# Lab-LVM/imagenet-models

Measured on AMD Instinct MI355X. Metric: images/sec (whole node) GA-ConvNeXt-T 3x224x224 bf16 training step, higher is better.
Workload: dtype bf16; 1 GPU; ga_convnext_tiny_768 train step (fwd + GA loss lam=-0.8 + bwd + all-reduce + adamw lr=0), batch 256/GPU, drop_path 0.2, synthetic 3x224x224; global_batch=256, parallelism=dp1, dist_backend=none, grad_exchange=torch, allreduce_buckets=0

## Files before the change

imagenet-models_amd/_lib.py:

```python
import ctypes as C
import os

_HERE = os.path.dirname(os.path.abspath(__file__))
LIB_PATH = os.environ.get('GAEXT_LIB') or os.path.join(_HERE, 'csrc', 'libgaext.so')

GA_F32, GA_BF16 = 0, 1
ACT_NONE, ACT_GELU, ACT_RELU = 0, 1, 2
A_PLAIN, A_PATCH2, A_STEM4_NCHW, A_CONV3, A_CONV3S2, A_NEIGH2 = 0, 1, 2, 3, 4, 5
C_PLAIN, C_UNPATCH2 = 0, 1

vp, i32, i64, f32 = C.c_void_p, C.c_int, C.c_int64, C.c_float


class GemmDesc(C.Structure):
    _fields_ = [
        ('M', i32), ('N', i32), ('K', i32), ('batch', i32), ('dtype', i32),
        ('A', vp), ('lda', i64), ('strideA', i64), ('a_batch_mod', i32), ('a_kind', i32),
        ('a_H', i32), ('a_W', i32), ('a_C', i32), ('a_act', i32),
        ('B', vp), ('ldb', i64), ('strideB', i64),
        ('C', vp), ('ldc', i64), ('strideC', i64), ('c_kind', i32),
        ('c_H', i32), ('c_W', i32), ('c_C', i32), ('c_f32', i32), ('C2', vp), ('c2_mode', i32),
        ('alpha', f32), ('bias', vp), ('strideBias', i64), ('act', i32),
        ('H', vp), ('ldh', i64), ('strideH', i64), ('h_is_deriv', i32),
        ('rowscale', vp), ('rows_per_scale', i32),
# ... 82 lines not shown
    'ga_unset_knob': ([C.c_char_p], i32),
    'ga_config_string': ([C.c_char_p, C.c_size_t], i32),
    'ga_gemm': ([C.POINTER(GemmDesc), vp], i32),
    'ga_wgrad': ([C.POINTER(WgradDesc), vp], i32),
    'ga_weight_prep': ([C.POINTER(WprepDesc), vp], i32),
    'ga_bias_fold': ([vp, vp, vp, vp, vp, vp, i32, i32, vp], i32),
    'ga_weight_unfold': ([C.POINTER(WunfoldDesc), vp], i32),
    'ga_dwconv7_fwd': ([vp, vp, vp, vp, i32, i32, i32, i32, i32, vp], i32),
    'ga_dwconv7_bwd_data': ([vp, vp, vp, vp, i32, i32, i32, i32, i32, vp], i32),
    'ga_dwconv7_bwd_data2': ([vp, vp, vp, vp, vp, vp, i32, i32, i32, i32, i32, vp], i32),
    'ga_dwconv7_bwd_weight': ([vp, vp, vp, vp, i32, i32, i32, i32, i32, vp, C.c_size_t, vp], i32),
    'ga_dwconv7_bwd_weight_workspace': ([i32, i32, i32, i32, i32], C.c_size_t),
    'ga_dwconv3_fwd': ([vp, vp, vp, i32, i32, i32, i32, i32, vp, vp, i32, vp], i32),
    'ga_dwconv3_bwd_data': ([vp, vp, vp, i32, i32, i32, i32, i32, i32, vp], i32),
    'ga_dwconv3_bwd_weight': ([vp, vp, vp, i32, i32, i32, i32, i32, i32, vp, C.c_size_t, vp], i32),
    'ga_dwconv3_bwd_weight_workspace': ([i32, i32, i32, i32, i32, i32], C.c_size_t),
    'ga_maxpool3s2_fwd': ([vp, vp, vp, i32, i32, i32, i32, i32, vp], i32),
    'ga_maxpool3s2_bwd': ([vp, vp, vp, i32, i32, i32, i32, i32, i32, vp], i32),
    'ga_bn_gelu_fwd': ([vp, vp, vp, vp, i64, i32, i32, vp], i32),
    'ga_bn_gelu_bwd_workspace': ([i64, i32], C.c_size_t),
    'ga_bn_gelu_bwd_reduce': ([vp, vp, vp, vp, vp, vp, vp, vp, i64, i32, i32, vp, C.c_size_t, vp], i32),
    'ga_bn_gelu_bwd_apply': ([vp, vp, vp, vp, vp, vp, vp, vp, vp, i64, vp, i64, i32, i32, vp], i32),
    'ga_se_bn_fwd': ([vp, i32, vp, vp, vp, vp, vp, vp, vp, vp, vp, vp, vp, vp, vp, vp, i32, i32, i32, i32, vp], i32),
    'ga_se_bn_bwd': ([vp, vp, vp, vp, vp, vp, vp, vp, i32, vp, vp, vp, vp, vp, vp, vp, vp, vp, vp, vp, vp, vp, vp, vp, vp, vp, vp, vp,
                      vp, vp, i32, i32, i32, vp], i32),
    'ga_se_residual_fwd': ([vp, vp, vp, vp, vp, vp, vp, vp, vp, i32, i32, i32, i32, vp], i32),
    'ga_se_residual_bwd_a': ([vp, vp, vp, vp, vp, vp, vp, vp, i32, i32, i32, i32, vp], i32),
    'ga_se_residual_bwd_b': ([vp, vp, vp, vp, vp, vp, vp, vp, vp, vp, vp, i32, i32, i32, i32, vp], i32),
    'ga_subsample2_fwd': ([vp, vp, i32, i32, i32, i32, i32, vp], i32),
    'ga_subsample2_bwd': ([vp, vp, i32, i32, i32, i32, i32, i32, vp], i32),
    'ga_wgrad_workspace': ([C.POINTER(WgradDesc)], C.c_size_t),
    'ga_gemm_form': ([C.POINTER(GemmDesc), C.c_char_p, C.c_size_t], i32),
    'ga_wgrad_form': ([C.POINTER(WgradDesc), C.c_char_p, C.c_size_t], i32),
    'ga_layernorm_fwd': ([vp, vp, vp, vp, vp, vp, i64, i32, f32, i32, vp], i32),
    'ga_layernorm_bwd': ([vp, vp, vp, vp, vp, vp, vp, vp, vp, i64, i32, i32, i32, vp], i32),
    'ga_layernorm_bwd_dp': ([vp, vp, vp, vp, vp, vp, vp, vp, vp, i64, i32, i32, vp, vp, i64, i32, vp], i32),
    'ga_bn_finalize': ([vp, vp, i64, vp, vp, f32, f32, vp, vp, vp, vp, vp, vp, i32, i32, vp], i32),
    'ga_affine_act': ([vp, vp, vp, vp, vp, i64, vp, i64, i32, i32, i32, i64, vp], i32),
    'ga_bn_bwd_reduce': ([vp, vp, vp, vp, vp, vp, i64, vp, vp, i64, i32, i32, i64, vp], i32),
    'ga_bn_bwd_apply': ([vp, vp, vp, vp, vp, vp, vp, vp, vp, i64, i64, vp, i64, i32, i32, i64, i64, vp], i32),
    'ga_pool_concat_fwd': ([vp, vp, i32, i32, i32, i32, i32, i32, i32, i32, i32, i32, vp], i32),
    'ga_pool_concat_bwd': ([vp, vp, vp, i32, i32, i32, i32, i32, i32, i32, i32, i32, i32, vp], i32),
    'ga_spatial_sum': ([vp, vp, vp, i32, i32, i32, f32, i32, vp], i32),
    'ga_se_mlp_fwd': ([vp, vp, vp, vp, vp, vp, vp, i32, i32, i32, vp], i32),
    'ga_se_mlp_bwd': ([vp, vp, vp, vp, vp, vp, vp, f32, vp, vp, vp, vp, i32, i32, i32, vp], i32),
    'ga_chan_scale': ([vp, vp, vp, vp, i32, i32, i32, i32, vp], i32),
    'ga_gram_pack_fwd': ([vp, vp, vp, i32, i32, i32, i32, i32, vp], i32),
    'ga_gram_pack_bwd': ([vp, vp, vp, vp, i32, i32, i32, i32, i32, vp], i32),
    'ga_gram_f64_fwd_workspace': ([i32, i32], C.c_size_t),
    'ga_gram_f64_bwd_workspace': ([i32, i32], C.c_size_t),
    'ga_gram_f64_fwd': ([vp, vp, vp, vp, C.c_size_t, i32, i32, i32, i32, i32, i32, i32, vp], i32),
    'ga_gram_f64_bwd': ([vp, vp, vp, vp, vp, vp, C.c_size_t, i32, i32, i32, i32, i32, i32, i32, vp], i32),
    'ga_token_cat': ([vp, vp, vp, i32, i32, i32, i32, vp], i32),
    'ga_token_split': ([vp, vp, vp, i32, i32, i32, i32, i32, i32, vp], i32),
    'ga_class_attn_fwd': ([vp, vp, vp, vp, i32, i32, i32, i32, f32, i32, vp], i32),
    'ga_class_attn_bwd': ([vp, vp, vp, vp, vp, vp, i32, i32, i32, i32, f32, i32, vp], i32),
    'ga_class_attn_fwd2': ([vp, vp, vp, i64, vp, vp, i32, i32, i32, i32, f32, i32, vp], i32),
    'ga_class_attn_bwd2': ([vp, vp, vp, vp, i64, vp, vp, vp, vp, i32, i32, i32, i32, f32, i32, vp], i32),
    'ga_loss_fwd_bwd': ([vp, vp, vp, vp, i32, i32, i32, f32, i32, f32, f32, i32, vp], i32),
    'ga_heads_topk': ([vp, i32, i32, i32, i32, vp, vp, vp], i32),
    'ga_sgd_step': ([vp, vp, vp, vp, i64, i32, f32, vp], i32),
    'ga_adamw_step': ([vp, vp, vp, vp, vp, i64, f32, vp], i32),
    'ga_weight_prep_batch': ([vp, i32, vp], i32),
    'ga_weight_unfold_batch': ([vp, i32, vp], i32),
    'ga_small_batch': ([vp, i32, vp], i32),
    'ga_cswin_attn_fwd': ([C.POINTER(CswinAttnDesc), vp], i32),
# ... 157 lines not shown
```

imagenet-models_amd/csrc/gemm.hip:

```cpp
#include <stdlib.h>
#include <algorithm>
#include <type_traits>
#include "common.h"
#include "gemm_select.h"

namespace {

constexpr int kThreads = 256;
constexpr int kRowBytes = 128;

__device__ __forceinline__ int xcd_remap(int bid, int nwg) {
    const int q = nwg >> 3, r = nwg & 7, xcd = bid & 7, idx = bid >> 3;
    return (xcd < r ? xcd * (q + 1) : r * (q + 1) + (xcd - r) * q) + idx;
}

struct RowCtx {
    long base;
    int y, x;
    bool valid;
};

__device__ __forceinline__ RowCtx make_row(int kind, long m, long M, long ld, int H, int W, int C) {
    RowCtx r;
    r.valid = m < M;
// ... 1717 lines not shown
                }
            }
    if (do_bias) {
#pragma unroll
        for (int tn = 0; tn < 8; ++tn) {
            float v = bsum[tn];
            v += __shfl_xor(v, 16, 64);
            v += __shfl_xor(v, 32, 64);
            const int n = n0 + wn * 128 + tn * 16 + lane;
            if (lane < 16 && n < d.N) atomicAdd(d.dbias + z * d.strideDbias + n, v * d.alpha);
        }
    }
}

__global__ __launch_bounds__(256) void tn2_reduce_kernel(const float* __restrict__ part, int nsplit, long nk, int K,
                                                         float alpha, float* __restrict__ dW, long ldw, long strideW) {
    const long z = blockIdx.y;
    const float* p = part + z * nsplit * nk;
    for (long i = ((long)blockIdx.x * 256 + threadIdx.x) * 4; i < nk; i += (long)gridDim.x * 1024) {
        float4 a = *reinterpret_cast<const float4*>(p + i);
#pragma unroll 4
        for (int s = 1; s < nsplit; ++s) {
            const float4 b = *reinterpret_cast<const float4*>(p + (long)s * nk + i);
            a.x += b.x; a.y += b.y; a.z += b.z; a.w += b.w;
        }
        const long n = i / K, k = i - n * K;
        float* dst = dW + z * strideW + n * ldw + k;
        dst[0] += alpha * a.x; dst[1] += alpha * a.y; dst[2] += alpha * a.z; dst[3] += alpha * a.w;
    }
}

using namespace gasel;

Knobs current_knobs() {
    Knobs k;
#define GA_SEL_KNOB(NAME) k.NAME = GA_KNOB(#NAME, Knobs{}.NAME)
    GA_SEL_KNOB(NT_R3); GA_SEL_KNOB(NT_R3_NEIGH2); GA_SEL_KNOB(NT_R3_CONV3S2); GA_SEL_KNOB(NT_PP); GA_SEL_KNOB(NT_PP_MINK);
    GA_SEL_KNOB(NT_BIG); GA_SEL_KNOB(NT_DMA); GA_SEL_KNOB(NT_DMA2); GA_SEL_KNOB(NT_DMA2_MINK); GA_SEL_KNOB(NT_T256);
    GA_SEL_KNOB(TN2); GA_SEL_KNOB(TN2_PATCH2); GA_SEL_KNOB(TN2_WGS); GA_SEL_KNOB(TN2_PART_MIN);
    GA_SEL_KNOB(CONV3_DIRECT); GA_SEL_KNOB(CONV0_DIRECT); GA_SEL_KNOB(STEM4_WGRAD_DIRECT);
#undef GA_SEL_KNOB
    return k;
}

int lds_error(int bytes) {
    ga_set_error("ga_gemm: cannot reserve %d bytes of LDS", bytes);
    return GA_ERR_HIP;
}

template <typename T, int TNW, int NWM, bool PLAIN, bool PRE, int EPI, bool DMA = false>
int launch_nt_(const ga_gemm_desc* d, hipStream_t s) {
    using CF = NTCfg<TNW, NWM>;
    constexpr int smem = DMA ? CF::SMEM_DMA : CF::SMEM;
    auto kern = gemm_nt_kernel<T, TNW, NWM, PLAIN, PRE, EPI, DMA>;
    static const int per_cu = [&] {
        int n = 0;
        if (smem > 65536 && hipFuncSetAttribute(reinterpret_cast<const void*>(kern),
                                                hipFuncAttributeMaxDynamicSharedMemorySize, smem) != hipSuccess)
            return 0;
        if (hipOccupancyMaxActiveBlocksPerMultiprocessor(&n, kern, CF::NTHR, smem) != hipSuccess || n < 1) n = 1;
        return n;
    }();
    if (per_cu == 0) return lds_error(smem);
    const int tiles = cdiv(d->M, CF::BM) * cdiv(d->N, CF::BN);
    const int cap = std::max(8, (per_cu * ga_num_cus() / d->batch) / 8 * 8);
    dim3 grid(std::min(tiles, cap), 1, d->batch), block(CF::NTHR);
    hipLaunchKernelGGL(kern, grid, block, smem, s, *d);
    return ga_check_launch("ga_gemm");
}

template <int EPI>
int launch_nt_pp(const ga_gemm_desc* d, hipStream_t s) {
    auto kern = gemm_nt_pp_kernel<EPI>;
    static const bool ok = hipFuncSetAttribute(reinterpret_cast<const void*>(kern), hipFuncAttributeMaxDynamicSharedMemorySize, kPPSmem) == hipSuccess;
    if (!ok) return lds_error(kPPSmem);
    const int tiles = cdiv(d->M, 256) * cdiv(d->N, 256);
// ... 174 lines not shown
```

imagenet-models_amd/csrc/gemm_select.h:

```cpp
#pragma once
#include <stddef.h>
#include <stdint.h>
#include <stdio.h>
#include <algorithm>
#include "../../include/gaext.h"

void ga_set_error(const char* fmt, ...);
bool ga_conv3_c64_eligible(const ga_gemm_desc* d);
bool ga_conv0_c8_eligible(const ga_gemm_desc* d);
int ga_conv3_c64_wgrad_wgs(const ga_wgrad_desc* d, int num_cus);
int ga_conv3s2_c64_wgrad_wgs(const ga_wgrad_desc* d, int num_cus);
int ga_conv0_c8_wgrad_wgs(const ga_wgrad_desc* d, int num_cus);
int ga_stem4_wgrad_wgs(const ga_wgrad_desc* d, int num_cus);

namespace gasel {

enum { EPI_GENERIC = -1, EPI_PLAIN = 0, EPI_FC1 = 1, EPI_FC2 = 2, EPI_DG2 = 3 };

struct Knobs {
    int NT_R3 = -1, NT_R3_NEIGH2 = 1, NT_R3_CONV3S2 = 1, NT_PP = -1, NT_PP_MINK = 512, NT_BIG = -1, NT_DMA = 1, NT_DMA2 = 10,
        NT_DMA2_MINK = 256, NT_T256 = -1;
    int TN2 = 1, TN2_PATCH2 = 1, TN2_WGS = 0, TN2_PART_MIN = 65536;
    int CONV3_DIRECT = 1, CONV0_DIRECT = 1, STEM4_WGRAD_DIRECT = 1;
};

inline int ceil_div(long a, long b) { return (int)((a + b - 1) / b); }
inline uintptr_t addr(const void* p) { return reinterpret_cast<uintptr_t>(p); }
inline bool aligned16(const void* p) { return (addr(p) & 15) == 0; }

#define GA_SEL_REQUIRE(cond, ...) \
    do { if (!(cond)) { ga_set_error(__VA_ARGS__); return GA_ERR_BAD_ARG; } } while (0)

inline int nt_validate(const ga_gemm_desc* d) {
    GA_SEL_REQUIRE(d && d->A && d->B && d->C, "ga_gemm: null operand");
    GA_SEL_REQUIRE(d->M > 0 && d->N > 0 && d->K > 0 && d->batch >= 1, "ga_gemm: bad shape M=%d N=%d K=%d batch=%d", d->M,
                   d->N, d->K, d->batch);
    GA_SEL_REQUIRE(d->dtype == GA_F32 || d->dtype == GA_BF16, "ga_gemm: bad dtype %d", d->dtype);
    const int epc = d->dtype == GA_BF16 ? 8 : 4;
    GA_SEL_REQUIRE(aligned16(d->A) && aligned16(d->B) && aligned16(d->C), "ga_gemm: operands must be 16-byte aligned");
    GA_SEL_REQUIRE(d->ldb % epc == 0 && d->strideB % epc == 0, "ga_gemm: ldb/strideB must be multiples of %d", epc);
    GA_SEL_REQUIRE(d->K % epc == 0, "ga_gemm: K=%d must be a multiple of %d (pad the operand)", d->K, epc);
    if (d->a_kind == GA_A_PLAIN) {
        GA_SEL_REQUIRE(d->lda % epc == 0 && d->strideA % epc == 0, "ga_gemm: lda/strideA must be multiples of %d", epc);
    } else if (d->a_kind == GA_A_PATCH2) {
        GA_SEL_REQUIRE(d->a_C % epc == 0 && d->a_H % 2 == 0 && d->a_W % 2 == 0 && d->K == 4 * d->a_C &&
                           (long)d->M % ((d->a_H / 2) * (d->a_W / 2)) == 0,
                       "ga_gemm: PATCH2 needs C%%%d==0, even H,W, K==4C", epc);
    } else if (d->a_kind == GA_A_CONV3) {
        GA_SEL_REQUIRE(d->a_C % epc == 0 && d->K == 9 * d->a_C && (long)d->M % (d->a_H * d->a_W) == 0,
                       "ga_gemm: CONV3 needs C%%%d==0, K==9C", epc);
    } else if (d->a_kind == GA_A_CONV3S2) {
        GA_SEL_REQUIRE(d->a_C % epc == 0 && d->K == 9 * d->a_C && (long)d->M % (((d->a_H + 1) / 2) * ((d->a_W + 1) / 2)) == 0,
                       "ga_gemm: CONV3S2 needs C%%%d==0, K==9C", epc);
    } else if (d->a_kind == GA_A_NEIGH2) {
        GA_SEL_REQUIRE(d->a_C % epc == 0 && d->K == 4 * d->a_C && (long)d->M % (d->a_H * d->a_W) == 0,
                       "ga_gemm: NEIGH2 needs C%%%d==0, K==4C", epc);
    } else if (d->a_kind == GA_A_STEM4_NCHW) {
// ... 206 lines not shown
    const long nk = (long)d->N * d->K;
    const long nk_min = k.TN2_PART_MIN;
    return (split > 1 && nk >= nk_min) ? (size_t)d->batch * split * nk * sizeof(float) : 0;
}

inline TnSel tn_select(const ga_wgrad_desc* d, int num_cus, const Knobs& k) {
    const bool has_ws = d->workspace != nullptr;
    int wgs;
    size_t need;
    auto direct = [&](int form, size_t per_wg) -> TnSel {
        need = (size_t)wgs * per_wg * sizeof(float);
        if (has_ws && (size_t)d->ws_bytes >= need) return {form, wgs, need, true};
        return {TN_TN, d->split_m, need, false};
    };
    if (k.CONV3_DIRECT && (wgs = ga_conv3_c64_wgrad_wgs(d, num_cus))) return direct(TN_CONV3_DIRECT, 64 * 576);
    if (k.CONV3_DIRECT && (wgs = ga_conv3s2_c64_wgrad_wgs(d, num_cus))) return direct(TN_CONV3S2_DIRECT, 64 * 576);
    if (k.CONV0_DIRECT && (wgs = ga_conv0_c8_wgrad_wgs(d, num_cus))) return direct(TN_CONV0_DIRECT, 64 * 72);
    if (k.STEM4_WGRAD_DIRECT && (wgs = ga_stem4_wgrad_wgs(d, num_cus))) return direct(TN_STEM4_DIRECT, (size_t)d->N * 49);
    if (tn2_eligible(d, k)) {
        int split;
        need = tn2_plan(d, num_cus, k, &split);
        return {TN_TN2, split, need, need && has_ws && (size_t)d->ws_bytes >= need};
    }
    return {TN_TN, d->split_m, 0, false};
}

inline void tn_form_name(const ga_wgrad_desc* d, const TnSel& s, char* buf, size_t n) {
    const char* const form[] = {"conv3_wgrad_direct", "conv3s2_wgrad_direct", "conv0_wgrad_direct", "stem4_wgrad_direct", "tn2", "tn"};
    if (s.form == TN_TN) snprintf(buf, n, "tn");
    else if (s.form != TN_TN2) snprintf(buf, n, "%s:wgs%d", form[s.form], s.split);
    else snprintf(buf, n, "tn2%s:split%d:%s", d->x_kind == GA_A_PATCH2 ? "p" : "", s.split, s.partials ? "partials" : "atomics");
}

#undef GA_SEL_REQUIRE

}
```

imagenet-models_amd/ops.py:

```python
import ctypes as C
import numbers
import os

import torch

from . import _lib as L
from ._lib import (A_CONV3, A_CONV3S2, A_NEIGH2, A_PATCH2, A_PLAIN, A_STEM4_NCHW, ACT_GELU, ACT_NONE, ACT_RELU, C_PLAIN, C_UNPATCH2,
                   GA_BF16, GA_F32)


def ga_dtype(t):
    if isinstance(t, torch.dtype):
        dt = t
    else:
        dt = t.dtype
    if dt == torch.bfloat16:
        return GA_BF16
    if dt == torch.float32:
        return GA_F32
    raise TypeError(f'unsupported dtype {dt}')


def torch_dtype(ga):
    return torch.bfloat16 if ga == GA_BF16 else torch.float32
# ... 291 lines not shown
        if apend:
            ajoin()

    def __len__(self):
        return len(self.calls)

    def mark(self, name):
        self.marks[name] = len(self.calls)

    def run_range(self, start, end, stream=None):
        self.finalize()
        s = current_stream_ptr() if stream is None else stream
        if any(self.lanes[start:end]):
            return self._run_lanes(start, end)
        for fn, args, label in self.calls[start:end]:
            rc = fn(*args, s)
            if rc != 0:
                L.check(rc, f'{self.name}:{label}')

    def gemm(self, A, B, Cout, M, N, K, dtype, lda=None, ldb=None, ldc=None, batch=1, strideA=0, strideB=0, strideC=0,
             a_batch_mod=0, a_kind=A_PLAIN, a_dims=(0, 0, 0), a_act=ACT_NONE, c_kind=C_PLAIN, c_dims=(0, 0, 0),
             c_f32=False, alpha=1.0, bias=None, strideBias=0, act=ACT_NONE, H=None, ldh=0, strideH=0, rowscale=None,
             rows_per_scale=1, R=None, ldr=0, strideR=0, relu_after=False, colsum=None, colsumsq=None, strideCol=0,
             C2=None, c2_mode=0, h_is_deriv=False, label=None):
        d = _set(L.GemmDesc(), M=M, N=N, K=K, batch=batch, dtype=dtype,
                 A=A, lda=(K if lda is None else lda), strideA=strideA, a_batch_mod=a_batch_mod, a_kind=a_kind, a_act=a_act,
                 B=B, ldb=(K if ldb is None else ldb), strideB=strideB,
                 C=Cout, ldc=(N if ldc is None else ldc), strideC=strideC, c_kind=c_kind, c_f32=c_f32, C2=C2, c2_mode=c2_mode,
                 h_is_deriv=h_is_deriv, alpha=alpha, bias=bias, strideBias=strideBias, act=act, H=H, ldh=ldh, strideH=strideH,
                 rowscale=rowscale, rows_per_scale=rows_per_scale, R=R, ldr=ldr, strideR=strideR, relu_after=relu_after,
                 colsum=colsum, colsumsq=colsumsq, strideCol=strideCol)
        d.a_H, d.a_W, d.a_C = a_dims
        d.c_H, d.c_W, d.c_C = c_dims
        self.record('ga_gemm', d, label=label)

    def attn_desc(self, qkv, out, lse, B, N, H, hd, scale, dtype, ldq=None, ldo=None):
        return _set(L.AttnDesc(), B=B, N=N, H=H, hd=hd, scale=scale, dtype=dtype, qkv=qkv, ldq=(3 * H * hd if ldq is None else ldq),
                    out=out, ldo=(H * hd if ldo is None else ldo), lse=lse)

    def attn_fwd(self, d, label=None):
        self.record('ga_attn_fwd', d, label=label)

    def attn_bwd(self, d, dout, dqkv, ws, label=None):
        self.record('ga_attn_bwd', d, dout, dqkv, ws, _nbytes(ws), label=label)

    def patchify(self, x, out, P, dtype, label=None):
        B, CH, H, W = x.shape
        self.record('ga_patchify', x, out, B, CH, H, W, P, dtype, label=label)

    def patchify_strided(self, x, out, P, S, dtype, label=None):
        B, CH, H, W = x.shape
        self.record('ga_patchify_strided', x, out, B, CH, H, W, P, S, dtype, label=label)

    def pos_add_fwd(self, tok, pos, x0, B, Np, Cdim, dtype, label=None):
        self.record('ga_pos_add_fwd', tok, pos, x0, B, Np, Cdim, dtype, label=label)

    def pos_add_bwd(self, dx0, dpos, B, Np, Cdim, dtype, label=None):
        self.record('ga_pos_add_bwd', dx0, dpos, B, Np, Cdim, dtype, label=label)

    def dwpool_fwd(self, x, w, bias, y, B, H, W_, Cin, mult, dtype, label=None):
        self.record('ga_dwpool_fwd', x, w, bias, y, B, H, W_, Cin, mult, dtype, label=label)

    def dwpool_bwd_data(self, dy, w, dx, B, H, W_, Cin, mult, dtype, label=None):
        self.record('ga_dwpool_bwd_data', dy, w, dx, B, H, W_, Cin, mult, dtype, label=label)

    def dwpool_bwd_weight(self, dy, x, dw, db, B, H, W_, Cin, mult, dtype, label=None):
        self.record('ga_dwpool_bwd_weight', dy, x, dw, db, B, H, W_, Cin, mult, dtype, label=label)
# ... 52 lines not shown
    def mlp_fwd(self, X, W1, b1, W2, b2, Y, M, Cdim, dtype, ldw1=None, ldw2=None, R=None, rowscale=None, rows_per_scale=1, label=None):
        H = 4 * Cdim
        d = _set(L.MlpDesc(), X=X, ldx=Cdim, W1=W1, ldw1=(Cdim if ldw1 is None else ldw1), b1=b1, W2=W2, ldw2=(H if ldw2 is None else ldw2),
                 b2=b2, R=R, ldr=Cdim, rowscale=rowscale, rows_per_scale=rows_per_scale, Y=Y, ldy=Cdim, M=M, C=Cdim, H=H, dtype=dtype)
        self.record('ga_mlp_fwd', d, label=label)

    def mlp_bwd(self, X, DY, W1, b1, W2T, W1T, A, DH, DX, M, Cdim, dtype, ldw1=None, ldw2t=None, ldw1t=None, label=None,
                dW1=None, db1=None, partials=None, max_blocks=0):
        H = 4 * Cdim
        d = _set(L.MlpBwdDesc(), X=X, ldx=Cdim, DY=DY, lddy=Cdim, W1=W1, ldw1=(Cdim if ldw1 is None else ldw1), b1=b1,
                 W2T=W2T, ldw2t=(Cdim if ldw2t is None else ldw2t), W1T=W1T, ldw1t=(H if ldw1t is None else ldw1t),
                 A=A, lda=H, DH=DH, lddh=H, DX=DX, lddx=Cdim, M=M, C=Cdim, H=H, dtype=dtype)
        if dW1 is not None:
            assert dW1.dtype == torch.float32 and db1 is not None and db1.dtype == torch.float32 and partials is not None
            assert dW1.stride(-1) == 1 and partials.dtype == torch.float32 and partials.is_contiguous()
            _set(d, dW1=dW1, ldw=dW1.stride(0), db1=db1, partials=partials, partials_bytes=partials.numel() * 4, max_blocks=max_blocks)
        self.record('ga_mlp_bwd', d, label=label)

    def wgrad(self, Y, X, dW, M, N, K, dtype, ldy=None, ldx=None, ldw=None, batch=1, strideY=0, strideX=0, strideW=0,
              x_kind=A_PLAIN, x_dims=(0, 0, 0), x_act=ACT_NONE, dbias=None, strideDbias=0, alpha=1.0, split_m=None,
              accumulate=True, x_batch_mod=0, label=None):
        if split_m is None:
            split_m = pick_split_m(M, N, K, batch, dtype)
        d = _set(L.WgradDesc(), M=M, N=N, K=K, batch=batch, dtype=dtype, Y=Y, ldy=(N if ldy is None else ldy), strideY=strideY,
                 X=X, ldx=(K if ldx is None else ldx), strideX=strideX, x_kind=x_kind, x_batch_mod=x_batch_mod, x_act=x_act,
                 dW=dW, ldw=(K if ldw is None else ldw), strideW=strideW, dbias=dbias, strideDbias=strideDbias, alpha=alpha,
                 split_m=split_m, accumulate=accumulate)
        d.x_H, d.x_W, d.x_C = x_dims
        need = self.lib.ga_wgrad_workspace(C.byref(d))
        if need:
            def patch(ptr, nbytes, d=d):
                d.workspace, d.ws_bytes = ptr, nbytes
            self._want_workspace(int(need), patch)
        self.record('ga_wgrad', d, label=label)

    def weight_prep(self, w, G, Co, Ci, KH, KW, dtype, out=None, ldo=0, outT=None, ldt=0, rs=None, cs=None, flip=False,
                    stem=False, row_perm=None, t_cols=0, label=None):
        d = _set(L.WprepDesc(), w=w, G=G, Co=Co, Ci=Ci, KH=KH, KW=KW, rs=rs, cs=cs, row_perm=row_perm, dtype=dtype,
                 out=out, ldo=ldo, outT=outT, ldt=ldt, flip=flip, stem=stem, t_cols=t_cols)
        if self.defer:
            return self._defer('wprep', d)
        self.record('ga_weight_prep', d, label=label)

    def bias_fold(self, W, b, rs, v, be, N, Cdim, row_perm=None, label=None):
        if self.defer:
            return self._small(kind=2, y=be, x=W, R=N, C=Cdim, b=b, rs=rs, v=v, row_perm=row_perm)
        self.record('ga_bias_fold', W, b, rs, v, row_perm, be, N, Cdim, label=label)

    def weight_unfold(self, G, ldg, N, Ci, KH=1, KW=1, gb=None, W=None, b=None, rs=None, cs=None, v=None, stem=False, dW=None,
                      db=None, d_rs=None, d_cs=None, d_v=None, row_perm=None, label=None):
        d = _set(L.WunfoldDesc(), G=G, ldg=ldg, gb=gb, W=W, b=b, rs=rs, cs=cs, v=v, row_perm=row_perm, N=N, Ci=Ci, KH=KH, KW=KW,
                 stem=stem, dW=dW, db=db, d_rs=d_rs, d_cs=d_cs, d_v=d_v)
        if self.defer:
            return self._defer('unfold', d)
        self.record('ga_weight_unfold', d, label=label)

    def dwconv7_fwd(self, x, w49, bias, y, B, H, W, Cdim, dtype, label=None):
        self.record('ga_dwconv7_fwd', x, w49, bias, y, B, H, W, Cdim, dtype, label=label)

    def dwconv7_bwd_data(self, dy, w49, res, dx, B, H, W, Cdim, dtype, dx2=None, scale2=None, label=None):
        if dx2 is not None:
            return self.record('ga_dwconv7_bwd_data2', dy, w49, res, dx, dx2, scale2, B, H, W, Cdim, dtype, label=label)
        self.record('ga_dwconv7_bwd_data', dy, w49, res, dx, B, H, W, Cdim, dtype, label=label)

    def dwconv7_bwd_weight(self, dy, x, dw49, dbias, B, H, W, Cdim, dtype, label=None):
        need = int(self.lib.ga_dwconv7_bwd_weight_workspace(B, H, W, Cdim, dtype))
        self._record_ws('ga_dwconv7_bwd_weight', need, dy, x, dw49, dbias, B, H, W, Cdim, dtype, label=label)
# ... 316 lines not shown
    def cast_to_f32(self, src, dst, n, dtype, label=None):
        self.record('ga_cast_to_f32', src, dst, n, dtype, label=label)

    def zero(self, t, label=None):
        self.record('ga_memset', t, 0, _nbytes(t), label=label or 'zero')


def mlp_supported(Cdim, H, dtype):
    return bool(L.load().ga_mlp_supported(Cdim, H, dtype))


def mlp_bwd_wgrad_supported(Cdim, H, dtype):
    return bool(L.load().ga_mlp_bwd_wgrad_supported(Cdim, H, dtype))


def mlp_bwd_partials(M, Cdim, dtype, max_blocks=0):
    d = L.MlpBwdDesc()
    d.M, d.C, d.H, d.dtype, d.max_blocks = M, Cdim, 4 * Cdim, dtype, max_blocks
    return int(L.load().ga_mlp_bwd_partials(C.byref(d)))


def gemm_form(d):
    buf = C.create_string_buffer(64)
    L.check(L.load().ga_gemm_form(C.byref(d), buf, 64), 'ga_gemm_form')
    return buf.value.decode()


def wgrad_form(d):
    buf = C.create_string_buffer(64)
    L.check(L.load().ga_wgrad_form(C.byref(d), buf, 64), 'ga_wgrad_form')
    return buf.value.decode()


def cswin_attn_bwd_workspace(d):
    return int(L.load().ga_cswin_attn_bwd_workspace(C.byref(d)))


def zero_(t):
    L.check(L.load().ga_memset(_ptr(t), 0, t.numel() * t.element_size(), current_stream_ptr()), 'ga_memset')
    return t


_NUM_CU = None


def num_cus():
    global _NUM_CU
    if _NUM_CU is None:
        n = C.c_int(256)
        L.check(L.load().ga_device_info(C.byref(n), None, None), 'ga_device_info')
        _NUM_CU = n.value
    return _NUM_CU


def pick_split_m(M, N, K, batch, dtype):
    slab = 64 if dtype == GA_BF16 else 32
    tiles = ((N + 127) // 128) * ((K + 127) // 128) * batch
    want = max(1, (2 * 256) // tiles)
    return int(max(1, min(want, (M + 4 * slab - 1) // (4 * slab))))
```

include/gaext.h:

```cpp
#ifndef GAEXT_H
#define GAEXT_H
#include <stddef.h>
#include <stdint.h>

#ifdef __cplusplus
extern "C" {
#endif

typedef void* ga_stream_t;

enum { GA_F32 = 0, GA_BF16 = 1 };
enum { GA_OK = 0, GA_ERR_BAD_ARG = -1, GA_ERR_UNSUPPORTED = -2, GA_ERR_HIP = -3 };

enum { GA_ACT_NONE = 0, GA_ACT_GELU = 1, GA_ACT_RELU = 2 };

enum {
    GA_A_PLAIN = 0,
    GA_A_PATCH2 = 1,
    GA_A_STEM4_NCHW = 2,
    GA_A_CONV3 = 3,
    GA_A_CONV3S2 = 4,
    GA_A_NEIGH2 = 5
};
enum {
// ... 43 lines not shown
    float* colsum;
    float* colsumsq;
    int64_t strideCol;
} ga_gemm_desc;
int ga_gemm(const ga_gemm_desc* d, ga_stream_t stream);

typedef struct {
    int M, N, K;
    int batch;
    int dtype;
    const void* Y;
    int64_t ldy, strideY;
    const void* X;
    int64_t ldx, strideX;
    int x_batch_mod;
    int x_kind;
    int x_H, x_W, x_C;
    int x_act;
    float* dW;
    int64_t ldw, strideW;
    float* dbias;
    int64_t strideDbias;
    float alpha;
    int split_m;
    int accumulate;
    void* workspace;
    int64_t ws_bytes;
} ga_wgrad_desc;
int ga_wgrad(const ga_wgrad_desc* d, ga_stream_t stream);
size_t ga_wgrad_workspace(const ga_wgrad_desc* d);

int ga_gemm_form(const ga_gemm_desc* d, char* buf, size_t n);
int ga_wgrad_form(const ga_wgrad_desc* d, char* buf, size_t n);

typedef struct {
    const float* w;
    int G, Co, Ci, KH, KW;
    const float* rs;
    const float* cs;
    const int* row_perm;
    int dtype;
    void* out;  int64_t ldo;
    void* outT; int64_t ldt;
    int flip;
    int stem;
    int t_cols;
} ga_wprep_desc;
int ga_weight_prep(const ga_wprep_desc* d, ga_stream_t stream);
int ga_bias_fold(const float* W, const float* b, const float* rs, const float* v, const int* row_perm, float* be, int N,
                 int C, ga_stream_t stream);
typedef struct {
    const float* G; int64_t ldg;
    const float* gb;
    const float* W; const float* b;
    const float* rs; const float* cs; const float* v;
    const int* row_perm;
    int N, Ci, KH, KW;
    int stem;
    float* dW; float* db; float* d_rs; float* d_cs; float* d_v;
} ga_wunfold_desc;
int ga_weight_unfold(const ga_wunfold_desc* d, ga_stream_t stream);

int ga_dwconv7_fwd(const void* x, const float* w49, const float* bias, void* y, int B, int H, int W, int C,
                   int dtype, ga_stream_t stream);
int ga_dwconv7_bwd_data(const void* dy, const float* w49, const void* res, void* dx, int B, int H, int W, int C,
                        int dtype, ga_stream_t stream);
// ... 328 lines not shown
```

Before: 10920 images/sec.

## Add split-K few-row GEMM and wgrad kernels for small-M launches

Adds dedicated bf16 NT and TN kernels for GEMMs with few rows (M up to 512). The NT kernel splits K across four waves and reduces partial sums in LDS; the TN kernel uses 64x64 output tiles. Both are selected only when the regular tiling would fill less than half the CUs, to raise parallelism for small head-layer GEMMs. The trade-off is an extra kernel path, extra host-side form queries while recording, and reliance on atomics for the column-sum and bias reductions.

```diff
diff --git a/imagenet-models_amd/_lib.py b/imagenet-models_amd/_lib.py
--- a/imagenet-models_amd/_lib.py
+++ b/imagenet-models_amd/_lib.py
@@ -138,6 +138,10 @@
     'ga_wgrad_workspace': ([C.POINTER(WgradDesc)], C.c_size_t),
     'ga_gemm_form': ([C.POINTER(GemmDesc), C.c_char_p, C.c_size_t], i32),
     'ga_wgrad_form': ([C.POINTER(WgradDesc), C.c_char_p, C.c_size_t], i32),
+    'ga_gemm_fewrows': ([C.POINTER(GemmDesc), vp], i32),
+    'ga_wgrad_fewrows': ([C.POINTER(WgradDesc), vp], i32),
+    'ga_gemm_fewrows_form': ([C.POINTER(GemmDesc), C.c_char_p, C.c_size_t], i32),
+    'ga_wgrad_fewrows_form': ([C.POINTER(WgradDesc), C.c_char_p, C.c_size_t], i32),
     'ga_layernorm_fwd': ([vp, vp, vp, vp, vp, vp, i64, i32, f32, i32, vp], i32),
     'ga_layernorm_bwd': ([vp, vp, vp, vp, vp, vp, vp, vp, vp, i64, i32, i32, i32, vp], i32),
     'ga_layernorm_bwd_dp': ([vp, vp, vp, vp, vp, vp, vp, vp, vp, i64, i32, i32, vp, vp, i64, i32, vp], i32),
diff --git a/imagenet-models_amd/csrc/gemm.hip b/imagenet-models_amd/csrc/gemm.hip
--- a/imagenet-models_amd/csrc/gemm.hip
+++ b/imagenet-models_amd/csrc/gemm.hip
@@ -1773,16 +1773,20 @@
 
 using namespace gasel;
 
-Knobs current_knobs() {
+}
+
+gasel::Knobs gasel::current_knobs() {
     Knobs k;
 #define GA_SEL_KNOB(NAME) k.NAME = GA_KNOB(#NAME, Knobs{}.NAME)
     GA_SEL_KNOB(NT_R3); GA_SEL_KNOB(NT_R3_NEIGH2); GA_SEL_KNOB(NT_R3_CONV3S2); GA_SEL_KNOB(NT_PP); GA_SEL_KNOB(NT_PP_MINK);
     GA_SEL_KNOB(NT_BIG); GA_SEL_KNOB(NT_DMA); GA_SEL_KNOB(NT_DMA2); GA_SEL_KNOB(NT_DMA2_MINK); GA_SEL_KNOB(NT_T256);
     GA_SEL_KNOB(TN2); GA_SEL_KNOB(TN2_PATCH2); GA_SEL_KNOB(TN2_WGS); GA_SEL_KNOB(TN2_PART_MIN);
-    GA_SEL_KNOB(CONV3_DIRECT); GA_SEL_KNOB(CONV0_DIRECT); GA_SEL_KNOB(STEM4_WGRAD_DIRECT);
+    GA_SEL_KNOB(CONV3_DIRECT); GA_SEL_KNOB(CONV0_DIRECT); GA_SEL_KNOB(STEM4_WGRAD_DIRECT); GA_SEL_KNOB(FEWROWS); GA_SEL_KNOB(FEWROWS_MAXM);
 #undef GA_SEL_KNOB
     return k;
 }
+
+namespace {
 
 int lds_error(int bytes) {
     ga_set_error("ga_gemm: cannot reserve %d bytes of LDS", bytes);
diff --git a/imagenet-models_amd/csrc/gemm_fewrows.hip b/imagenet-models_amd/csrc/gemm_fewrows.hip
--- /dev/null
+++ b/imagenet-models_amd/csrc/gemm_fewrows.hip
@@ -0,0 +1,365 @@
+#include <algorithm>
+#include "common.h"
+#include "gemm_select.h"
+
+namespace {
+
+using namespace gasel;
+
+constexpr int kFrThreads = 256;
+constexpr int kFrChunk = 4;
+
+__device__ __forceinline__ uint4 fr_zero4() { return make_uint4(0u, 0u, 0u, 0u); }
+
+struct FrFrag {
+    uint4 a[2][kFrChunk], b[2][kFrChunk];
+};
+
+__global__ __launch_bounds__(kFrThreads) void gemm_nt_fewrows_kernel(const ga_gemm_desc d) {
+    __shared__ __attribute__((aligned(16))) float part[4][32 * 32];
+    const int tid = threadIdx.x, lane = tid & 63, wave = tid >> 6;
+    const int tiles_n = (d.N + 31) >> 5;
+    const int tile_m = blockIdx.x / tiles_n, tile_n = blockIdx.x - tile_m * tiles_n;
+    const int m0 = tile_m * 32, n0 = tile_n * 32;
+    const long z = blockIdx.z;
+    const long za = d.a_batch_mod > 0 ? z % d.a_batch_mod : z;
+    const bf16_t* Ab = reinterpret_cast<const bf16_t*>(d.A) + za * d.strideA;
+    const bf16_t* Bb = reinterpret_cast<const bf16_t*>(d.B) + z * d.strideB;
+
+    const int fr = lane & 15, kq = (lane >> 4) * 8;
+    const bf16_t* Ap[2];
+    const bf16_t* Bp[2];
+#pragma unroll
+    for (int i = 0; i < 2; ++i) {
+        Ap[i] = Ab + (long)min(m0 + 16 * i + fr, d.M - 1) * d.lda;
+        Bp[i] = Bb + (long)min(n0 + 16 * i + fr, d.N - 1) * d.ldb;
+    }
+    const int nsteps = (d.K + 31) >> 5, per = (nsteps + 3) >> 2;
+    const int s0 = wave * per, s1 = min(s0 + per, nsteps);
+    const int nchunks = s1 > s0 ? (s1 - s0 + kFrChunk - 1) / kFrChunk : 0;
+
+    auto load = [&](int c, FrFrag& f) {
+#pragma unroll
+        for (int i = 0; i < kFrChunk; ++i) {
+            const int s = s0 + c * kFrChunk + i, k = s * 32 + kq;
+            const bool ok = s < s1 && k < d.K;
+            const int kk = ok ? k : 0;
+#pragma unroll
+            for (int j = 0; j < 2; ++j) {
+                const uint4 va = *reinterpret_cast<const uint4*>(Ap[j] + kk);
+                const uint4 vb = *reinterpret_cast<const uint4*>(Bp[j] + kk);
+                f.a[j][i] = ok ? va : fr_zero4();
+                f.b[j][i] = ok ? vb : fr_zero4();
+            }
+        }
+    };
+    f32x4_t acc[2][2];
+#pragma unroll
+    for (int i = 0; i < 2; ++i)
+#pragma unroll
+        for (int j = 0; j < 2; ++j) acc[i][j] = f32x4_t{0.f, 0.f, 0.f, 0.f};
+    auto mma = [&](const FrFrag& f) {
+#pragma unroll
+        for (int i = 0; i < kFrChunk; ++i)
+#pragma unroll
+            for (int bn = 0; bn < 2; ++bn)
+#pragma unroll
+                for (int bm = 0; bm < 2; ++bm)
+                    acc[bn][bm] = __builtin_amdgcn_mfma_f32_16x16x32_bf16(*reinterpret_cast<const bf16x8_t*>(&f.b[bn][i]),
+                                                                          *reinterpret_cast<const bf16x8_t*>(&f.a[bm][i]),
+                                                                          acc[bn][bm], 0, 0, 0);
+    };
+    FrFrag f0, f1;
+    if (nchunks > 0) load(0, f0);
+    for (int c = 0; c < nchunks; c += 2) {
+        if (c + 1 < nchunks) load(c + 1, f1);
+        mma(f0);
+        if (c + 1 < nchunks) {
+            if (c + 2 < nchunks) load(c + 2, f0);
+            mma(f1);
+        }
+    }
+
+#pragma unroll
+    for (int bn = 0; bn < 2; ++bn)
+#pragma unroll
+        for (int bm = 0; bm < 2; ++bm) {
+            const int row = bm * 16 + (lane & 15), c4 = bn * 4 + (lane >> 4);
+            *reinterpret_cast<f32x4_t*>(&part[wave][row * 32 + ((c4 ^ (row & 7)) << 2)]) = acc[bn][bm];
+        }
+    __syncthreads();
+
+    const int row = tid >> 3, c4 = tid & 7;
+    const long m = m0 + row;
+    const int n = n0 + c4 * 4;
+    float v[4];
+    {
+        const int o = row * 32 + ((c4 ^ (row & 7)) << 2);
+        const f32x4_t p0 = *reinterpret_cast<const f32x4_t*>(&part[0][o]), p1 = *reinterpret_cast<const f32x4_t*>(&part[1][o]);
+        const f32x4_t p2 = *reinterpret_cast<const f32x4_t*>(&part[2][o]), p3 = *reinterpret_cast<const f32x4_t*>(&part[3][o]);
+#pragma unroll
+        for (int j = 0; j < 4; ++j) v[j] = (p0[j] + p1[j]) + (p2[j] + p3[j]);
+    }
+    const bool live = m < d.M && n < d.N;
+    const bool full = n + 3 < d.N;
+    float cs[4] = {0.f, 0.f, 0.f, 0.f}, cq[4] = {0.f, 0.f, 0.f, 0.f};
+    if (live) {
+        const float* bias = d.bias ? d.bias + z * d.strideBias : nullptr;
+#pragma unroll
+        for (int j = 0; j < 4; ++j) v[j] = v[j] * d.alpha + ((bias && n + j < d.N) ? bias[n + j] : 0.f);
+        const long coff = z * d.strideC + m * d.ldc + n;
+        if (d.act == GA_ACT_GELU) {
+            float w[4];
+#pragma unroll
+            for (int j = 0; j < 4; ++j) gelu_both_fast(v[j], v[j], w[j]);
+            if (d.C2) {
+                bf16_t* C2p = reinterpret_cast<bf16_t*>(d.C2) + coff;
+                if (full) {
+                    store4(C2p, w);
+                } else {
+#pragma unroll
+                    for (int j = 0; j < 4; ++j)
+                        if (n + j < d.N) C2p[j] = f2bf(w[j]);
+                }
+            }
+        }
+        if (d.H) {
+            const bf16_t* Hp = reinterpret_cast<const bf16_t*>(d.H) + z * d.strideH + m * d.ldh + n;
+            float h[4] = {0.f, 0.f, 0.f, 0.f};
+            if (full) {
+                load4(Hp, h);
+            } else {
+#pragma unroll
+                for (int j = 0; j < 4; ++j)
+                    if (n + j < d.N) h[j] = bf2f(Hp[j]);
+            }
+#pragma unroll
+            for (int j = 0; j < 4; ++j) v[j] *= h[j];
+        }
+        if (d.rowscale) {
+            const float s = d.rowscale[(unsigned)m / (unsigned)d.rows_per_scale];
+#pragma unroll
+            for (int j = 0; j < 4; ++j) v[j] *= s;
+        }
+        if (d.R) {
+            const bf16_t* Rp = reinterpret_cast<const bf16_t*>(d.R) + z * d.strideR + m * d.ldr + n;
+            float r[4] = {0.f, 0.f, 0.f, 0.f};
+            if (full) {
+                load4(Rp, r);
+            } else {
+#pragma unroll
+                for (int j = 0; j < 4; ++j)
+                    if (n + j < d.N) r[j] = bf2f(Rp[j]);
+            }
+#pragma unroll
+            for (int j = 0; j < 4; ++j) v[j] += r[j];
+        }
+#pragma unroll
+        for (int j = 0; j < 4; ++j)
+            if (n + j < d.N) {
+                cs[j] = v[j];
+                cq[j] = v[j] * v[j];
+            }
+        if (d.c_f32) {
+            float* Cp = reinterpret_cast<float*>(d.C) + coff;
+            if (full) {
+                store4(Cp, v);
+            } else {
+#pragma unroll
+                for (int j = 0; j < 4; ++j)
+                    if (n + j < d.N) Cp[j] = v[j];
+            }
+        } else {
+            bf16_t* Cp = reinterpret_cast<bf16_t*>(d.C) + coff;
+            if (full) {
+                store4(Cp, v);
+            } else {
+#pragma unroll
+                for (int j = 0; j < 4; ++j)
+                    if (n + j < d.N) Cp[j] = f2bf(v[j]);
+            }
+        }
+    }
+    if (d.colsum) {
+        const bool sq = d.colsumsq != nullptr;
+#pragma unroll
+        for (int j = 0; j < 4; ++j) {
+#pragma unroll
+            for (int o = 8; o < 64; o <<= 1) {
+                cs[j] += __shfl_xor(cs[j], o, 64);
+                cq[j] += __shfl_xor(cq[j], o, 64);
+            }
+        }
+        __syncthreads();
+        float* red = &part[0][0];
+        if (lane < 8) {
+#pragma unroll
+            for (int j = 0; j < 4; ++j) {
+                red[wave * 32 + lane * 4 + j] = cs[j];
+                red[128 + wave * 32 + lane * 4 + j] = cq[j];
+            }
+        }
+        __syncthreads();
+        if (tid < 64) {
+            const int which = tid >> 5, col = tid & 31;
+            if (n0 + col < d.N && (which == 0 || sq)) {
+                const float* r = red + which * 128 + col;
+                const float s = (r[0] + r[32]) + (r[64] + r[96]);
+                atomicAdd((which ? d.colsumsq : d.colsum) + z * d.strideCol + n0 + col, s);
+            }
+        }
+    }
+}
+
+constexpr int kFrTnRows = 128;
+constexpr int kFrTnRowBytes = 256;
+
+__device__ __forceinline__ int fr_tn_swz(int row) { return ((row & 3) << 1) | (((row >> 3) & 1) << 3); }
+
+__global__ __launch_bounds__(kFrThreads) void gemm_tn_fewrows_kernel(const ga_wgrad_desc d) {
+    __shared__ __attribute__((aligned(16))) unsigned char img[kFrTnRows * kFrTnRowBytes];
+    const int tid = threadIdx.x, lane = tid & 63, wave = tid >> 6;
+    const int wn = wave >> 1, wk = wave & 1;
+    const int tiles_k = (d.K + 63) >> 6;
+    const int tile_n = blockIdx.x / tiles_k, tile_k = blockIdx.x - tile_n * tiles_k;
+    const int n0 = tile_n * 64, k0 = tile_k * 64;
+    const long z = blockIdx.z;
+    const long zx = d.x_batch_mod > 0 ? z % d.x_batch_mod : z;
+    const bf16_t* Yb = reinterpret_cast<const bf16_t*>(d.Y) + z * d.strideY;
+    const bf16_t* Xb = reinterpret_cast<const bf16_t*>(d.X) + zx * d.strideX;
+
+    const int cc = tid & 15, rr = tid >> 4;
+    const bool is_y = cc < 8;
+    const int col = is_y ? n0 + cc * 8 : k0 + (cc - 8) * 8;
+    const bool col_ok = is_y ? col < d.N : col < d.K;
+    const bf16_t* src = col_ok ? (is_y ? Yb + col : Xb + col) : Yb;
+    const long ld = col_ok ? (is_y ? d.ldy : d.ldx) : d.ldy;
+    const bool do_bias = d.dbias != nullptr && tile_k == 0;
+    uint4 rg[8];
+    float bsum[8];
+#pragma unroll
+    for (int j = 0; j < 8; ++j) bsum[j] = 0.f;
+
+    auto g_load = [&](int slab) {
+#pragma unroll
+        for (int i = 0; i < 8; ++i) {
+            const long m = (long)slab * kFrTnRows + rr + 16 * i;
+            const uint4 t = *reinterpret_cast<const uint4*>(src + (m < d.M ? m : d.M - 1) * ld);
+            rg[i] = (col_ok && m < d.M) ? t : fr_zero4();
+        }
+    };
+    auto s_store = [&]() {
+#pragma unroll
+        for (int i = 0; i < 8; ++i) {
+            const int row = rr + 16 * i;
+            *reinterpret_cast<uint4*>(img + row * kFrTnRowBytes + ((cc ^ fr_tn_swz(row)) << 4)) = rg[i];
+            if (do_bias && is_y) {
+                float y[8];
+                unpack8(rg[i], y);
+#pragma unroll
+                for (int j = 0; j < 8; ++j) bsum[j] += y[j];
+            }
+        }
+    };
+
+    f32x4_t acc[2][2];
+#pragma unroll
+    for (int i = 0; i < 2; ++i)
+#pragma unroll
+        for (int j = 0; j < 2; ++j) acc[i][j] = f32x4_t{0.f, 0.f, 0.f, 0.f};
+
+    const int nslabs = (d.M + kFrTnRows - 1) / kFrTnRows;
+    g_load(0);
+    for (int s = 0; s < nslabs; ++s) {
+        s_store();
+        __syncthreads();
+        if (s + 1 < nslabs) g_load(s + 1);
+        const int rows = min(kFrTnRows, d.M - s * kFrTnRows);
+#pragma unroll
+        for (int ks = 0; ks < kFrTnRows / 32; ++ks) {
+            if (ks * 32 >= rows) break;
+            s16x4_t yf[2][2], xf[2][2];
+#pragma unroll
+            for (int hf = 0; hf < 2; ++hf) {
+                const int row = ks * 32 + 8 * (lane >> 4) + 4 * hf + ((lane & 15) >> 2);
+                const int sw = fr_tn_swz(row);
+#pragma unroll
+                for (int t = 0; t < 2; ++t) {
+                    const int ch_y = ((wn * 32 + t * 16) >> 3) + ((lane & 3) >> 1);
+                    const int ch_x = 8 + ((wk * 32 + t * 16) >> 3) + ((lane & 3) >> 1);
+                    const unsigned ay = row * kFrTnRowBytes + ((ch_y ^ sw) << 4) + 8 * (lane & 1);
+                    const unsigned ax = row * kFrTnRowBytes + ((ch_x ^ sw) << 4) + 8 * (lane & 1);
+                    yf[t][hf] = __builtin_amdgcn_ds_read_tr16_b64_v4i16((__attribute__((address_space(3))) s16x4_t*)(img + ay));
+                    xf[t][hf] = __builtin_amdgcn_ds_read_tr16_b64_v4i16((__attribute__((address_space(3))) s16x4_t*)(img + ax));
+                }
+            }
+#pragma unroll
+            for (int tn = 0; tn < 2; ++tn)
+#pragma unroll
+                for (int tk = 0; tk < 2; ++tk)
+                    acc[tn][tk] = __builtin_amdgcn_mfma_f32_16x16x32_bf16(*reinterpret_cast<const bf16x8_t*>(&yf[tn][0]),
+                                                                          *reinterpret_cast<const bf16x8_t*>(&xf[tk][0]),
+                                                                          acc[tn][tk], 0, 0, 0);
+        }
+        __syncthreads();
+    }
+
+    float* W = d.dW + z * d.strideW;
+#pragma unroll
+    for (int tn = 0; tn < 2; ++tn)
+#pragma unroll
+        for (int tk = 0; tk < 2; ++tk)
+#pragma unroll
+            for (int r = 0; r < 4; ++r) {
+                const int n = n0 + wn * 32 + tn * 16 + (lane >> 4) * 4 + r;
+                const int k = k0 + wk * 32 + tk * 16 + (lane & 15);
+                if (n < d.N && k < d.K) {
+                    const float v = acc[tn][tk][r] * d.alpha;
+                    if (d.accumulate) atomicAdd(W + (long)n * d.ldw + k, v);
+                    else W[(long)n * d.ldw + k] = v;
+                }
+            }
+    if (do_bias) {
+        float* red = reinterpret_cast<float*>(img);
+        if (is_y) {
+#pragma unroll
+            for (int j = 0; j < 8; ++j) red[rr * 64 + cc * 8 + j] = bsum[j];
+        }
+        __syncthreads();
+        if (tid < 64 && n0 + tid < d.N) {
+            float s = 0.f;
+            for (int r = 0; r < 16; ++r) s += red[r * 64 + tid];
+            atomicAdd(d.dbias + z * d.strideDbias + n0 + tid, s * d.alpha);
+        }
+    }
+}
+
+}
+
+extern "C" int ga_gemm_fewrows(const ga_gemm_desc* d, ga_stream_t stream) {
+    if (const int rc = nt_validate(d)) return rc;
+    if (!nt_fewrows_wanted(d, ga_num_cus(), current_knobs())) return ga_gemm(d, stream);
+    dim3 grid(cdiv(d->M, 32) * cdiv(d->N, 32), 1, d->batch), block(kFrThreads);
+    hipLaunchKernelGGL(gemm_nt_fewrows_kernel, grid, block, 0, reinterpret_cast<hipStream_t>(stream), *d);
+    return ga_check_launch("ga_gemm_fewrows");
+}
+
+extern "C" int ga_gemm_fewrows_form(const ga_gemm_desc* d, char* buf, size_t n) {
+    if (const int rc = nt_validate(d)) return rc;
+    if (buf && n) nt_fewrows_name(d, nt_fewrows_wanted(d, ga_num_cus(), current_knobs()), buf, n);
+    return GA_OK;
+}
+
+extern "C" int ga_wgrad_fewrows(const ga_wgrad_desc* d, ga_stream_t stream) {
+    if (const int rc = tn_validate(d)) return rc;
+    if (!tn_fewrows_wanted(d, ga_num_cus(), current_knobs())) return ga_wgrad(d, stream);
+    dim3 grid(cdiv(d->N, 64) * cdiv(d->K, 64), 1, d->batch), block(kFrThreads);
+    hipLaunchKernelGGL(gemm_tn_fewrows_kernel, grid, block, 0, reinterpret_cast<hipStream_t>(stream), *d);
+    return ga_check_launch("ga_wgrad_fewrows");
+}
+
+extern "C" int ga_wgrad_fewrows_form(const ga_wgrad_desc* d, char* buf, size_t n) {
+    if (const int rc = tn_validate(d)) return rc;
+    if (buf && n) snprintf(buf, n, "%s", tn_fewrows_wanted(d, ga_num_cus(), current_knobs()) ? "fewrows_tn64x64" : "none");
+    return GA_OK;
+}
diff --git a/imagenet-models_amd/csrc/gemm_select.h b/imagenet-models_amd/csrc/gemm_select.h
--- a/imagenet-models_amd/csrc/gemm_select.h
+++ b/imagenet-models_amd/csrc/gemm_select.h
@@ -22,7 +22,10 @@
         NT_DMA2_MINK = 256, NT_T256 = -1;
     int TN2 = 1, TN2_PATCH2 = 1, TN2_WGS = 0, TN2_PART_MIN = 65536;
     int CONV3_DIRECT = 1, CONV0_DIRECT = 1, STEM4_WGRAD_DIRECT = 1;
+    int FEWROWS = 1, FEWROWS_MAXM = 512;
 };
+
+Knobs current_knobs();
 
 inline int ceil_div(long a, long b) { return (int)((a + b - 1) / b); }
 inline uintptr_t addr(const void* p) { return reinterpret_cast<uintptr_t>(p); }
@@ -295,6 +298,35 @@
     else snprintf(buf, n, "tn2%s:split%d:%s", d->x_kind == GA_A_PATCH2 ? "p" : "", s.split, s.partials ? "partials" : "atomics");
 }
 
+
+inline bool nt_fewrows_wanted(const ga_gemm_desc* d, int num_cus, const Knobs& k) {
+    if (!k.FEWROWS || d->dtype != GA_BF16 || d->a_kind != GA_A_PLAIN || d->c_kind != GA_C_PLAIN || d->a_act != GA_ACT_NONE ||
+        d->relu_after)
+        return false;
+    if (d->act != GA_ACT_NONE ? classify_epilogue(d) != EPI_FC1 : d->C2 != nullptr) return false;
+    if (d->H && !d->h_is_deriv) return false;
+    if (d->colsumsq && !d->colsum) return false;
+    if (d->strideC % 4 != 0 || (d->R && d->strideR % 4 != 0) || (d->H && d->strideH % 4 != 0) || (d->bias && (addr(d->bias) & 3)))
+        return false;
+    if (d->M > k.FEWROWS_MAXM || d->batch > 65535) return false;
+    if (nt_select(d, num_cus, k).form != NT_STAGED) return false;
+    return (long)ceil_div(d->M, 128) * ceil_div(d->N, 32 * nt_tile_width(d->N)) * d->batch < num_cus / 2;
+}
+
+inline void nt_fewrows_name(const ga_gemm_desc* d, bool wanted, char* buf, size_t n) {
+    const char* const epi[] = {"generic", "plain", "fc1", "fc2", "dg2"};
+    if (wanted) snprintf(buf, n, "fewrows32x32:%s", epi[classify_epilogue(d) + 1]);
+    else snprintf(buf, n, "none");
+}
+
+inline bool tn_fewrows_wanted(const ga_wgrad_desc* d, int num_cus, const Knobs& k) {
+    if (!k.FEWROWS || d->dtype != GA_BF16 || d->x_kind != GA_A_PLAIN || d->x_act != GA_ACT_NONE) return false;
+    if (!d->accumulate && d->split_m > 1) return false;
+    if (d->M > k.FEWROWS_MAXM || d->batch > 65535) return false;
+    if (tn_select(d, num_cus, k).form != TN_TN) return false;
+    return (long)ceil_div(d->N, 128) * ceil_div(d->K, 128) * d->split_m * d->batch < num_cus / 2;
+}
+
 #undef GA_SEL_REQUIRE
 
 }
diff --git a/imagenet-models_amd/ops.py b/imagenet-models_amd/ops.py
--- a/imagenet-models_amd/ops.py
+++ b/imagenet-models_amd/ops.py
@@ -347,7 +347,7 @@
                  colsum=colsum, colsumsq=colsumsq, strideCol=strideCol)
         d.a_H, d.a_W, d.a_C = a_dims
         d.c_H, d.c_W, d.c_C = c_dims
-        self.record('ga_gemm', d, label=label)
+        self.record('ga_gemm' if gemm_fewrows_form(d) == 'none' else 'ga_gemm_fewrows', d, label=label or 'ga_gemm')
 
     def attn_desc(self, qkv, out, lse, B, N, H, hd, scale, dtype, ldq=None, ldo=None):
         return _set(L.AttnDesc(), B=B, N=N, H=H, hd=hd, scale=scale, dtype=dtype, qkv=qkv, ldq=(3 * H * hd if ldq is None else ldq),
@@ -466,7 +466,7 @@
             def patch(ptr, nbytes, d=d):
                 d.workspace, d.ws_bytes = ptr, nbytes
             self._want_workspace(int(need), patch)
-        self.record('ga_wgrad', d, label=label)
+        self.record('ga_wgrad' if wgrad_fewrows_form(d) == 'none' else 'ga_wgrad_fewrows', d, label=label or 'ga_wgrad')
 
     def weight_prep(self, w, G, Co, Ci, KH, KW, dtype, out=None, ldo=0, outT=None, ldt=0, rs=None, cs=None, flip=False,
                     stem=False, row_perm=None, t_cols=0, label=None):
@@ -849,6 +849,16 @@
     return buf.value.decode()
 
 
+def gemm_fewrows_form(d):
+    buf = C.create_string_buffer(64)
+    return buf.value.decode() if L.load().ga_gemm_fewrows_form(C.byref(d), buf, 64) == 0 else 'none'
+
+
+def wgrad_fewrows_form(d):
+    buf = C.create_string_buffer(64)
+    return buf.value.decode() if L.load().ga_wgrad_fewrows_form(C.byref(d), buf, 64) == 0 else 'none'
+
+
 def cswin_attn_bwd_workspace(d):
     return int(L.load().ga_cswin_attn_bwd_workspace(C.byref(d)))
 
diff --git a/include/gaext.h b/include/gaext.h
--- a/include/gaext.h
+++ b/include/gaext.h
@@ -99,6 +99,11 @@
 
 int ga_gemm_form(const ga_gemm_desc* d, char* buf, size_t n);
 int ga_wgrad_form(const ga_wgrad_desc* d, char* buf, size_t n);
+
+int ga_gemm_fewrows(const ga_gemm_desc* d, ga_stream_t stream);
+int ga_wgrad_fewrows(const ga_wgrad_desc* d, ga_stream_t stream);
+int ga_gemm_fewrows_form(const ga_gemm_desc* d, char* buf, size_t n);
+int ga_wgrad_fewrows_form(const ga_wgrad_desc* d, char* buf, size_t n);
 
 typedef struct {
     const float* w;
```

After: 11080 images/sec (median of 6 runs). 1.5% higher.
